# microsoft/StemGNN

Measured on AMD Instinct MI355X. Metric: forecast-steps/sec (train), higher is better.
Workload: dtype f32

## Files before the change

### stemgnn_amd/csrc/block.hip

```cpp
#include <hip/hip_runtime.h>

#include "../../include/stemgnn_hip.h"
#include "devattr.h"
#include "gemm2.h"
#include "gemm2s.h"
#include "gemm_core.h"
#include "layout.h"
#include "reduce.h"
#include "wgrad.h"
#include "heads.h"
#include "glu_fused.h"
#include "glu_fused_bf16.h"

#define SG_TRY(e)                                \
  do {                                           \
    hipError_t _e = (e);                         \
    if (_e != hipSuccess) return -(int)_e;       \
  } while (0)

__device__ __forceinline__ float sg_sigmoid(float v) { return __frcp_rn(1.f + __expf(-v)); }

struct SgDiv {
  unsigned d, magic;
  __device__ __forceinline__ int div(int x) const { return d == 1u ? x : (int)__umulhi((unsigned)x, magic); }
  __device__ __forceinline__ void divmod(int x, int& q, int& r) const { q = div(x); r = x - q * (int)d; }
};
static inline SgDiv sg_div(int d) {
  SgDiv v;
  v.d = (unsigned)d;
  v.magic = d > 1 ? (unsigned)((1ull << 32) / (unsigned)d + 1ull) : 0u;
  return v;
}
static inline bool sg_div_ok(long xmax, int d) { return d >= 1 && xmax >= 0 && (unsigned long long)xmax * (unsigned)d < (1ull << 32); }

struct XView {
  const float* p;
  long sb, sn, st;
  int N;
  __device__ __forceinline__ float at(int b, int n, int t) const { return p[b * sb + n * sn + t * st]; }
  __device__ __forceinline__ float row(int m, int t) const {
    const int b = m / N;
    return at(b, m - b * N, t);
  }
};

struct GftFwdOp {
  const float* T;
  XView X;
  float* G;
  int B, N, W;
  SgDiv dN, dW;
  __device__ bool setup(int, int& M, int& Nn, int& K0, int& K1) const {
    M = 3 * N; Nn = B * W; K0 = 0; K1 = N;
    return true;
  }
  __device__ float a(int, int i, int k) const { return T[(size_t)i * N + k]; }
  __device__ float b(int, int k, int j) const {
    int bb, t;
    dW.divmod(j, bb, t);
    return X.at(bb, k, t);
  }
  __device__ void epi(int, int i, int j, float v) const {
    int kq, n, bb, t;
    dN.divmod(i, kq, n);
    dW.divmod(j, bb, t);
    G[((size_t)bb * N + n) * (3 * W) + kq * W + t] = v;
  }
};

struct GftBwdDxOp {
  const float* T;
  const float* dG;
  float* dX;
  int B, N, W;
  size_t slab;
  SgDiv dN, dW;
  __device__ bool setup(int, int& M, int& Nn, int& K0, int& K1) const {
    M = N; Nn = B * W; K0 = 0; K1 = 3 * N;
    return true;
  }
  __device__ float a(int, int i, int k) const { return T[(size_t)k * N + i]; }
  __device__ float b(int, int k, int j) const {
    int kq, n, bb, t;
    dN.divmod(k, kq, n);
    dW.divmod(j, bb, t);
    const size_t o = ((size_t)bb * N + n) * (3 * W) + kq * W + t;
    return dG[o] + dG[o + slab];
  }
  __device__ void epi(int, int i, int j, float v) const {
    int bb, t;
    dW.divmod(j, bb, t);
    dX[((size_t)bb * N + i) * W + t] = v;
  }
};

struct GftBwdDtOp {
  const float* dG;
  XView X;
  float* dT;
  int B, N, W, accumulate;
  size_t slab;
  SgDiv dN, dW;
  __device__ bool setup(int, int& M, int& Nn, int& K0, int& K1) const {
    M = 3 * N; Nn = N; K0 = 0; K1 = B * W;
    return true;
  }
  __device__ float a(int, int i, int k) const {
    int kq, n, bb, t;
    dN.divmod(i, kq, n);
    dW.divmod(k, bb, t);
    const size_t o = ((size_t)bb * N + n) * (3 * W) + kq * W + t;
    return dG[o] + dG[o + slab];
  }
  __device__ float b(int, int k, int j) const {
    int bb, t;
    dW.divmod(k, bb, t);
    return X.at(bb, j, t);
  }
  __device__ void epi(int, int i, int j, float v) const {
    float* o = dT + (size_t)i * N + j;
    *o = accumulate ? (*o + v) : v;
  }
};

struct GftBwdDt2Op {
  const float* dG[2];
  XView X[2];
  float* dT;
  int B, N, W;
  size_t slab;
  SgDiv dN, dW;
  __device__ bool setup(int, int& M, int& Nn, int& K0, int& K1) const {
    M = 3 * N; Nn = N; K0 = 0; K1 = 2 * B * W;
    return true;
  }
  __device__ float a(int, int i, int k) const {
    const int blk = k >= B * W ? 1 : 0, kk = k - blk * B * W;
    int kq, n, bb, t;
    dN.divmod(i, kq, n);
    dW.divmod(kk, bb, t);
    const size_t o = ((size_t)bb * N + n) * (3 * W) + kq * W + t;
    const float* g = dG[blk];
    return g[o] + g[o + slab];
  }
  __device__ float b(int, int k, int j) const {
    const int blk = k >= B * W ? 1 : 0, kk = k - blk * B * W;
    int bb, t;
    dW.divmod(kk, bb, t);
    return X[blk].at(bb, j, t);
  }
  __device__ void epi(int, int i, int j, float v) const { dT[(size_t)i * N + j] = v; }
};

template <bool GATE = true>
struct GluFwdEpiT {
  static constexpr bool WHOLE = true;
  const float* bp[2];
  float* out[2];
  float* gate[2];
  int cp[2];
  template <int NI>
  __device__ void whole(int r, int, int row0, int col0, int M, int N, const sg_f32x16 (&acc)[NI][2], int lane) const {
    const bool hi = (lane & 16) != 0;
    const int k = lane & 15;
    const bool live0 = col0 < N, live1 = col0 + 32 < N;
    const float* b = bp[r];
    const float bl0 = live0 ? b[col0 + k] : 0.f, br0 = live0 ? b[col0 + 16 + k] : 0.f;
    const float bl1 = live1 ? b[col0 + 32 + k] : 0.f, br1 = live1 ? b[col0 + 48 + k] : 0.f;
    const bool live = hi ? live1 : live0;
    const int c = (col0 >> 1) + (lane & 31);
    float* po = out[r] + c;
    float* pg = GATE ? gate[r] + c : nullptr;
    const int ld = cp[r];
#pragma unroll
    for (int i = 0; i < NI; ++i) {
#pragma unroll
      for (int reg = 0; reg < 16; ++reg) {
        const float m0 = acc[i][0][reg], m1 = acc[i][1][reg];
        const float o0 = __shfl_xor(m0, 16, 64), o1 = __shfl_xor(m1, 16, 64);
        const float u = hi ? o1 + bl1 : m0 + bl0;
        const float v = hi ? m1 + br1 : o0 + br0;
        const float g = sg_sigmoid(v);
        const int row = row0 + i * 32 + g2_row_of(reg, lane);
        if (live && row < M) {
          po[(size_t)row * ld] = u * g;
          if constexpr (GATE) pg[(size_t)row * ld] = g;
        }
      }
    }
  }
};
using GluFwdEpi = GluFwdEpiT<true>;

struct GluDpreEpi {
  static constexpr bool WHOLE = true;
  const float* out[2];
  const float* gate[2];
  float* dpre[2];
  int cp;
  template <int NI>
  __device__ void whole(int r, int, int row0, int col0, int M, int N, const sg_f32x16 (&acc)[NI][2], int lane) const {
    const bool hi = (lane & 16) != 0;
    const float* po = out[r];
    const float* pg = gate[r];
    float* pd = dpre[r];
#pragma unroll
    for (int i = 0; i < NI; ++i) {
      float y[2][16], g[2][16];
#pragma unroll
      for (int j = 0; j < 2; ++j) {
        const int c = col0 + j * 32 + (lane & 31);
        const bool cl = c < N;
#pragma unroll
        for (int reg = 0; reg < 16; ++reg) {
          const int row = row0 + i * 32 + g2_row_of(reg, lane);
          const size_t o = (size_t)(row < M ? row : 0) * cp + (cl ? c : 0);
          y[j][reg] = po[o];
          g[j][reg] = pg[o];
        }
      }
#pragma unroll
      for (int j = 0; j < 2; ++j) {
        const int cb = col0 + j * 32;
        const bool cl = cb + (lane & 31) < N;
        const bool cl_lo = cb < N, cl_hi = cb + 16 < N;
        float* dp = pd + 2 * cb + (lane & 31);
#pragma unroll
        for (int reg = 0; reg < 16; ++reg) {
          const int row = row0 + i * 32 + g2_row_of(reg, lane);
          const float d = acc[i][j][reg];
          const float left = d * g[j][reg], right = d * y[j][reg] * (1.f - g[j][reg]);
          const float recv = __shfl_xor(hi ? left : right, 16, 64);
          if (row < M) {
            float* q = dp + (size_t)row * 2 * cp;
// ... 145 lines not shown
  __device__ float a(int, int i, int k) const {
    const float* p = k < Wm ? dpF + (size_t)i * Wm + k : dpB + (size_t)i * W + (k - Wm);
    return *p;
  }
  __device__ float b(int, int k, int j) const {
    const float* p = k < Wm ? Fw + (size_t)k * Wm + j : BCw + (size_t)(k - Wm) * Wm + j;
    return *p;
  }
  __device__ void epi(int, int i, int j, float v) const { dig[(size_t)i * Wm + j] = v; }
};

struct Da3Op {
  const float* dig;
  const float* wfold;
  const float* out[2];
  const float* gate[2];
  float* dpre[2];
  int cp2[2];
  int M, Wm, WmP;
  __device__ bool setup(int z, int& M_, int& N_, int& K0, int& K1) const {
    M_ = M; N_ = cp2[z]; K0 = 0; K1 = Wm;
    return true;
  }
  __device__ float a(int, int i, int k) const { return dig[(size_t)i * Wm + k]; }
  __device__ float b(int z, int k, int j) const { return wfold[(size_t)((z ? cp2[0] : 0) + j) * WmP + k]; }
  __device__ void epi(int z, int i, int j, float v) const {
    const size_t o = (size_t)i * cp2[z] + j;
    const float g = gate[z][o], y = out[z][o];
    float* dp = dpre[z] + (size_t)i * 2 * cp2[z] + ((j >> 4) << 5) + (j & 15);
    dp[0] = v * g;
    dp[16] = v * y * (1.f - g);
  }
};

struct HeadsWgradOp {
  const float *pa0[5], *pa1[5];
  int lda0[5], lda1[5], split[5], Mw[5], Nw[5], nb[5], rdiv[5], ldp[5], on[5];
  float sign[5];
  const float* pb[5];
  long sb[5], sn[5], st[5];
  float* part[5];
  int M, S, chunk;
  __device__ bool setup(int z, int& M_, int& N_, int& K0, int& K1) const {
    const int which = z / S, s = z - which * S;
    K0 = s * chunk; K1 = min(M, K0 + chunk);
    M_ = Mw[which]; N_ = Nw[which];
    return on[which] != 0;
  }
  __device__ float a(int z, int i, int k) const {
    const int w = z / S;
    const float *p0 = pa0[w], *p1 = pa1[w];
    const int l0 = lda0[w], l1 = lda1[w], sp = split[w];
    const float sg = sign[w];
    const bool lo = i < sp;
    const float* base = lo ? p0 : p1;
    const size_t off = (size_t)k * (lo ? l0 : l1) + (lo ? i : i - sp);
    return sg * base[off];
  }
  __device__ float b(int z, int k, int j) const {
    const int w = z / S;
    const int n = nb[w];
    const int kb = k / rdiv[w], kr = k - kb * rdiv[w];
    const float v = pb[w][kb * sb[w] + kr * sn[w] + (j < n ? j : n - 1) * st[w]];
    return j < n ? v : 1.f;
  }
  __device__ void epi(int z, int i, int j, float v) const {
    const int w = z / S, s = z - w * S;
    part[w][((size_t)s * Mw[w] + i) * ldp[w] + j] = v;
  }
};

constexpr int SG_LONG_K = 640;
constexpr int SG_WG_MAX_TILES = 256;
static inline bool wg_tiles_fit(WgGemm* q, int n) { return wg_tile_index(q, n) <= SG_WG_MAX_TILES; }
static inline int split_chunk(int M, int S) { return ((M + S - 1) / S + 15) & ~15; }

extern "C" int stemgnn_gft_fwd(const float* mul_L, const float* X, long xs_b, long xs_n, long xs_t,
                               float* G, int B, int N, int W, void* stream) {
  if (!mul_L || !X || !G || B <= 0 || N <= 0 || W <= 0) return SG_EINVAL;
  if (!sg_div_ok(3L * N + 64, N) || !sg_div_ok((long)B * W + 64, W)) return SG_EINVAL;
  GftFwdOp op{mul_L + (size_t)N * N, XView{X, xs_b, xs_n, xs_t, N}, G, B, N, W, sg_div(N), sg_div(W)};
  hipStream_t st = (hipStream_t)stream;
  if (N <= 512) {
    if (xs_n == 1) SG_TRY((sg_launch_gemm<GftFwdOp, 32, 32, true, true, false, 128, true>(op, 3 * N, B * W, 1, st)));
    else SG_TRY((sg_launch_gemm<GftFwdOp, 32, 32, true, false, false, 128, true>(op, 3 * N, B * W, 1, st)));
    return 0;
  }
  if (xs_n == 1) SG_TRY((sg_launch_gemm<GftFwdOp, 32, 64, true, true, false, 64, true>(op, 3 * N, B * W, 1, st)));
  else SG_TRY((sg_launch_gemm<GftFwdOp, 32, 64, true, false, false, 64, true>(op, 3 * N, B * W, 1, st)));
  return 0;
}

extern "C" int stemgnn_gft_bwd(const float* mul_L, const float* X, long xs_b, long xs_n, long xs_t,
                               const float* dG, float* dX, float* dmul_L, int accumulate,
                               int B, int N, int W, void* stream) {
  if (!mul_L || !X || !dG || (!dmul_L && !dX) || B <= 0 || N <= 0 || W <= 0) return SG_EINVAL;
  hipStream_t st = (hipStream_t)stream;
  const bool bk128 = N <= 512;
  if (!sg_div_ok(3L * N + 128, N) || !sg_div_ok((long)B * W + 128, W)) return SG_EINVAL;
  if (dX) {
    GftBwdDxOp op{mul_L + (size_t)N * N, dG, dX, B, N, W, (size_t)B * N * 3 * W, sg_div(N), sg_div(W)};
    if (bk128) SG_TRY((sg_launch_gemm<GftBwdDxOp, 32, 32, false, false, false, 128, true>(op, N, B * W, 1, st)));
    else SG_TRY((sg_launch_gemm<GftBwdDxOp, 32, 32, false, false, false, 64, true>(op, N, B * W, 1, st)));
  }
  if (!dmul_L) return 0;
  GftBwdDtOp op{dG, XView{X, xs_b, xs_n, xs_t, N}, dmul_L + (size_t)N * N, B, N, W, accumulate, (size_t)B * N * 3 * W, sg_div(N),
                sg_div(W)};
  if (bk128) {
    if (xs_t == 1) SG_TRY((sg_launch_gemm<GftBwdDtOp, 32, 32, true, true, false, 128, true>(op, 3 * N, N, 1, st)));
    else SG_TRY((sg_launch_gemm<GftBwdDtOp, 32, 32, true, false, false, 128, true>(op, 3 * N, N, 1, st)));
    return 0;
  }
  if (xs_t == 1) SG_TRY((sg_launch_gemm<GftBwdDtOp, 32, 32, true, true, false, 64, true>(op, 3 * N, N, 1, st)));
  else SG_TRY((sg_launch_gemm<GftBwdDtOp, 32, 32, true, false, false, 64, true>(op, 3 * N, N, 1, st)));
  return 0;
}

extern "C" int stemgnn_gft_bwd_dt2(const float* X0, long xs0_b, long xs0_n, long xs0_t, const float* dG0, const float* X1,
                                   long xs1_b, long xs1_n, long xs1_t, const float* dG1, float* dmul_L, int B, int N, int W,
                                   void* stream) {
  if (!X0 || !dG0 || !X1 || !dG1 || !dmul_L || B <= 0 || N <= 0 || W <= 0) return SG_EINVAL;
  hipStream_t st = (hipStream_t)stream;
  if (!sg_div_ok(3L * N + 128, N) || !sg_div_ok(2L * B * W + 128, W)) return SG_EINVAL;
  GftBwdDt2Op op{{dG0, dG1}, {XView{X0, xs0_b, xs0_n, xs0_t, N}, XView{X1, xs1_b, xs1_n, xs1_t, N}}, dmul_L + (size_t)N * N,
                 B, N, W, (size_t)B * N * 3 * W, sg_div(N), sg_div(W)};
  if (N <= 512) SG_TRY((sg_launch_gemm<GftBwdDt2Op, 32, 32, true, false, false, 128, true>(op, 3 * N, N, 1, st)));
  else SG_TRY((sg_launch_gemm<GftBwdDt2Op, 32, 32, true, false, false, 64, true>(op, 3 * N, N, 1, st)));
  return 0;
}

struct GluFwdBufs {
  const float* G;
  float* out[2][3];
  float* gate[2][3];
};
static GluFwdBufs glu_bufs_saved(const SgDims& d, float* saved) {
  const SgSavedLayout S = sg_saved_layout(d);
  GluFwdBufs b;
  b.G = saved + S.G;
  for (int r = 0; r < 2; ++r)
    for (int l = 0; l < 3; ++l) { b.out[r][l] = saved + S.out[r][l]; b.gate[r][l] = saved + S.gate[r][l]; }
  return b;
}
static GluFwdBufs glu_bufs_infer(const SgDims& d, float* ws, bool pp) {
  const SgInferLayout I = sg_infer_layout(d, pp);
  GluFwdBufs b;
  b.G = ws + I.G;
  for (int r = 0; r < 2; ++r) {
    b.out[r][0] = pp ? ws + I.pp[r][0] : nullptr;
    b.out[r][1] = pp ? ws + I.pp[r][1] : nullptr;
    b.out[r][2] = ws + I.out2[r];
    for (int l = 0; l < 3; ++l) b.gate[r][l] = nullptr;
  }
  return b;
}
template <bool INF>
static int glu_fwd_layers(const SgDims& d, const float* packed, const unsigned short* const* fpl, int splits,
                          const GluFwdBufs& bf, hipStream_t st) {
  const SgPackedLayout P = sg_packed_layout(d);
  using Epi = GluFwdEpiT<!INF>;
  for (int l = 0; l < 3; ++l) {
    G2Args g;
    G2SArgs gs;
    Epi e;
    for (int r = 0; r < 2; ++r) {
      g.A[r] = l == 0 ? bf.G : bf.out[r][l - 1];
      g.lda[r] = l == 0 ? d.KG : d.CP;
      g.B[r] = packed + P.w[r][l];
      g.ldb[r] = sg_glu_np(d, l, r);
      g.M[r] = d.M; g.N[r] = sg_glu_np(d, l, r); g.K[r] = sg_glu_kin(d, l);
      if (fpl) {
        gs.A[r] = g.A[r]; gs.lda[r] = g.lda[r]; gs.P[r] = fpl[r * 3 + l];
        gs.M[r] = g.M[r]; gs.N[r] = g.N[r]; gs.K[r] = g.K[r]; gs.Kp[r] = g2s_pad32(g.K[r]);
      }
      e.bp[r] = packed + P.b[r][l];
      e.out[r] = bf.out[r][l];
      e.gate[r] = bf.gate[r][l];
      e.cp[r] = sg_glu_cp(d, l, r);
    }
    g.nsplit = 1; g.chunk = (sg_glu_kin(d, l) + 15) & ~15; g.b_ones_col = -1;
    if (fpl && l > 0 && g2s_ok(gs, 2)) {
      SG_TRY((g2s_launch<Epi>(gs, e, 2, splits, st)));
      continue;
    }
    if (sg_glu_kin(d, l) > SG_LONG_K) SG_TRY((g2_launch<Epi, true, false, 64, true>(g, e, 2, st)));
    else SG_TRY((g2_launch<Epi, true, false, 64>(g, e, 2, st)));
  }
  return 0;
}

static int glu_fused_mode() {
  const char* ef = getenv("STEMGNN_GLU_FUSED");
  return ef ? atoi(ef) : 1;
}
static inline bool sg_aligned16(const void* p) { return (((uintptr_t)p) & 15) == 0; }
static bool glu_fwd_fused_ok(const SgDims& d, int fmode, const void* packed) {
  return gf_geom(d).ok && fmode != 0 && sg_aligned16(packed);
}
static bool glu_dgrad_fused_ok(const SgDims& d, int dmode, const void* packed, const void* scratch) {
  return gd_geom(d).ok && dmode != 0 && sg_aligned16(packed) && sg_aligned16(scratch);
}

template <bool INF = false>
static int glu_fwd_impl(const float* packed, const GluFwdBufs& bf, int B, int N, int W, int multi, void* stream, int m_pick,
                        bool fused_only) {
  if (!packed || !bf.G || B <= 0 || N <= 0 || W <= 0 || multi <= 0) return SG_EINVAL;
  const SgDims d = sg_dims(B, N, W, multi);
  const SgPackedLayout P = sg_packed_layout(d);
// ... 790 lines not shown
```

### stemgnn_amd/csrc/front.hip

```cpp
#include <hip/hip_runtime.h>
#include <stdlib.h>
#include <stdint.h>

#include "../../include/stemgnn_hip.h"
#include "dq_reduce.h"
#include "gemm_core.h"
#include "layout.h"

#define SG_TRY(e)                                \
  do {                                           \
    hipError_t _e = (e);                         \
    if (_e != hipSuccess) return -(int)_e;       \
  } while (0)

constexpr int ATTN_NBC = 8;

__device__ __forceinline__ void sg_philox4(uint64_t seed, uint64_t offset, uint64_t idx, uint32_t (&w)[4]) {
  uint32_t c0 = (uint32_t)idx, c1 = (uint32_t)(idx >> 32), c2 = (uint32_t)offset, c3 = (uint32_t)(offset >> 32);
  uint32_t k0 = (uint32_t)seed, k1 = (uint32_t)(seed >> 32);
#pragma unroll
  for (int r = 0; r < 10; ++r) {
    const uint32_t hi0 = __umulhi(0xD2511F53u, c0), lo0 = 0xD2511F53u * c0;
    const uint32_t hi1 = __umulhi(0xCD9E8D57u, c2), lo1 = 0xCD9E8D57u * c2;
    c0 = hi1 ^ c1 ^ k0; c1 = lo1; c2 = hi0 ^ c3 ^ k1; c3 = lo0;
    k0 += 0x9E3779B9u; k1 += 0xBB67AE85u;
  }
  w[0] = c0; w[1] = c1; w[2] = c2; w[3] = c3;
}
__device__ __forceinline__ int sg_drop_nq(int N) { return 64 * ((N + 255) >> 8); }
__device__ __forceinline__ bool sg_keep_word(uint32_t w, float p) { return (float)w * 2.3283064365386963e-10f >= p; }

__device__ __forceinline__ float sg_wave_sum(float v) {
#pragma unroll
  for (int o = 32; o > 0; o >>= 1) v += __shfl_xor(v, o, 64);
  return v;
}
__device__ __forceinline__ float sg_wave_max(float v) {
#pragma unroll
  for (int o = 32; o > 0; o >>= 1) v = fmaxf(v, __shfl_xor(v, o, 64));
  return v;
}
__device__ __forceinline__ float sg_lrelu(float v, float alpha) { return v > 0.f ? v : alpha * v; }

__global__ __launch_bounds__(256) void sg_keyquery_kernel(const float* __restrict__ h, const float* __restrict__ wk,
                                                          const float* __restrict__ wq, float* __restrict__ key,
                                                          float* __restrict__ query, int B, int N) {
  __shared__ float red[4][64][2];
  const int b = blockIdx.x, lane = threadIdx.x & 63, wave = threadIdx.x >> 6;
  const int i = blockIdx.y * 64 + lane;
  float ak = 0.f, aq = 0.f;
  if (i < N) {
    const float* hp = h + (size_t)b * N + i;
    const size_t stride = (size_t)B * N;
#pragma unroll 4
    for (int s = wave; s < N; s += 4) {
      const float v = hp[s * stride];
      ak = fmaf(v, wk[s], ak);
      aq = fmaf(v, wq[s], aq);
    }
  }
  red[wave][lane][0] = ak;
  red[wave][lane][1] = aq;
  __syncthreads();
  if (wave == 0 && i < N) {
    key[(size_t)b * N + i] = (red[0][lane][0] + red[1][lane][0]) + (red[2][lane][0] + red[3][lane][0]);
    query[(size_t)b * N + i] = (red[0][lane][1] + red[1][lane][1]) + (red[2][lane][1] + red[3][lane][1]);
  }
}

__global__ __launch_bounds__(256) void sg_attention_fwd_kernel(
    const float* __restrict__ key, const float* __restrict__ query, float alpha, float drop_p, int training,
    const uint64_t* __restrict__ seedp, int B, int N, int bn, float* __restrict__ rowsum, float* __restrict__ Apart,
    float* __restrict__ degpart) {
  extern __shared__ __attribute__((aligned(16))) float smem[];
  float* qmax = smem;
  const int lane = threadIdx.x & 63, wave = threadIdx.x >> 6;
  float* acc = smem + bn + wave * N;
  const int b0 = blockIdx.y * bn, b1 = min(B, b0 + bn);
  for (int b = b0 + wave; b < b1; b += 4) {
    float m = -INFINITY;
    for (int j = lane; j < N; j += 64) m = fmaxf(m, query[(size_t)b * N + j]);
    m = sg_wave_max(m);
    if (lane == 0) qmax[b - b0] = m;
  }
  __syncthreads();
  const int i = blockIdx.x * 4 + wave;
  if (i >= N) return;
  const bool drop = training && drop_p > 0.f;
  uint64_t seed = 0, offset = 0;
// ... 414 lines not shown
  __shared__ float red[4][2];
  const int s = blockIdx.x;
  const size_t BN = (size_t)B * N;
  float ak = 0.f, aq = 0.f;
  for (size_t e = threadIdx.x; e < BN; e += 256) {
    const float hv = h[(size_t)s * BN + e];
    ak = fmaf(dkey[e], hv, ak);
    aq = fmaf(dquery[e], hv, aq);
  }
  ak = sg_wave_sum(ak);
  aq = sg_wave_sum(aq);
  const int lane = threadIdx.x & 63, wave = threadIdx.x >> 6;
  if (lane == 0) { red[wave][0] = ak; red[wave][1] = aq; }
  __syncthreads();
  if (threadIdx.x == 0) {
    dwk[s] = (red[0][0] + red[1][0]) + (red[2][0] + red[3][0]);
    dwq[s] = (red[0][1] + red[1][1]) + (red[2][1] + red[3][1]);
  }
}

__global__ void sg_dropout_mask_kernel(float drop_p, const uint64_t* __restrict__ seedp, size_t n, int N, float* __restrict__ mask) {
  const size_t idx = (size_t)blockIdx.x * blockDim.x + threadIdx.x;
  if (idx >= n) return;
  const size_t row = idx / (size_t)N;
  const int j = (int)(idx - row * (size_t)N);
  uint32_t w[4];
  sg_philox4(seedp[0], seedp[1], row * sg_drop_nq(N) + (uint64_t)((j >> 8) * 64 + (j & 63)), w);
  mask[idx] = sg_keep_word(w[(j >> 6) & 3], drop_p) ? 1.f : 0.f;
}

struct ChebFwdOp {
  const float* L;
  const float* Bm;
  float* out;
  int N, sub;
  __device__ bool setup(int, int& M, int& Nn, int& K0, int& K1) const {
    M = N; Nn = N; K0 = 0; K1 = N;
    return true;
  }
  __device__ float a(int, int i, int k) const { return L[(size_t)i * N + k]; }
  __device__ float b(int, int k, int j) const { return Bm[(size_t)k * N + j]; }
  __device__ void epi(int, int i, int j, float v) const {
    const size_t o = (size_t)i * N + j;
    out[o] = sub ? 2.f * v - L[o] : 2.f * v;
  }
};

struct ChebBwd1Op {
  const float *L, *T2, *dT1, *dT2, *dT3;
  float *dLp, *dT2p;
  int N;
  __device__ bool setup(int, int& M, int& Nn, int& K0, int& K1) const {
    M = N; Nn = N; K0 = 0; K1 = N;
    return true;
  }
  __device__ float a(int z, int i, int k) const { return z == 0 ? dT3[(size_t)i * N + k] : L[(size_t)k * N + i]; }
  __device__ float b(int z, int k, int j) const { return z == 0 ? T2[(size_t)j * N + k] : dT3[(size_t)k * N + j]; }
  __device__ void epi(int z, int i, int j, float v) const {
    const size_t o = (size_t)i * N + j;
    if (z == 0) dLp[o] = dT1[o] - dT3[o] + 2.f * v;
    else dT2p[o] = dT2[o] + 2.f * v;
  }
};
struct ChebBwd2Op {
  const float *L, *dT2p, *dLp;
  float* dL;
  int N;
  __device__ bool setup(int, int& M, int& Nn, int& K0, int& K1) const {
    M = N; Nn = N; K0 = 0; K1 = 2 * N;
    return true;
  }
  __device__ float a(int, int i, int k) const {
    const float* p = k < N ? dT2p + (size_t)i * N + k : L + (size_t)(k - N) * N + i;
    return *p;
  }
  __device__ float b(int, int k, int j) const {
    const float* p = k < N ? L + (size_t)j * N + k : dT2p + (size_t)(k - N) * N + j;
    return *p;
  }
  __device__ void epi(int, int i, int j, float v) const {
    const size_t o = (size_t)i * N + j;
    dL[o] = dLp[o] + 2.f * v;
  }
};

extern "C" size_t stemgnn_attn_saved_floats(int B, int N) {
  return (size_t)3 * B * N + (size_t)N * N + N + (size_t)ATTN_NBC * N * N + (size_t)ATTN_NBC * N + B;
}
extern "C" size_t stemgnn_attn_scratch_floats(int B, int N, int nchunk) {
  return (size_t)N * N + (size_t)2 * B * N + (size_t)B * nchunk * N;
}

extern "C" int stemgnn_attn_laplacian_fwd(const float* h, const float* wk, const float* wq, float alpha,
                                          float drop_p, int training, const uint64_t* seed, int B, int N,
                                          float* saved, float* attention_out, float* mul_L, int parts, void* stream) {
  if (!h || !wk || !wq || !saved || !attention_out || !mul_L || B <= 0 || N <= 0 || (parts & 3) == 0) return SG_EINVAL;
  if (training && drop_p > 0.f && !seed) return SG_EINVAL;
  if (drop_p < 0.f || drop_p >= 1.f) return SG_EINVAL;
  hipStream_t st = (hipStream_t)stream;
  float* key = saved;
  float* query = key + (size_t)B * N;
  float* rowsum = query + (size_t)B * N;
  float* A = rowsum + (size_t)B * N;
  float* deg = A + (size_t)N * N;
  if (parts & 1) {
    hipLaunchKernelGGL(sg_keyquery_kernel, dim3(B, (N + 63) / 64), dim3(256), 0, st, h, wk, wq, key, query, B, N);
    SG_TRY(hipGetLastError());
    float* Apart = deg + N;
    float* degpart = Apart + (size_t)ATTN_NBC * N * N;
    const int nbc = B < ATTN_NBC ? B : ATTN_NBC;
    const int bn = (B + nbc - 1) / nbc;
    const size_t lds = (size_t)(bn + 4 * N) * sizeof(float);
    if (lds > 64 * 1024) return SG_EINVAL;
    hipLaunchKernelGGL(sg_attention_fwd_kernel, dim3((N + 3) / 4, (B + bn - 1) / bn), dim3(256), lds, st, key, query, alpha,
                       drop_p, training, seed, B, N, bn, rowsum, Apart, degpart);
    SG_TRY(hipGetLastError());
    if (parts & 2) {
      hipLaunchKernelGGL(sg_laplacian_fused_kernel, dim3((N + 31) / 32, (N + 31) / 32), dim3(256), 0, st, Apart, degpart,
                         (B + bn - 1) / bn, B, N, A, deg, attention_out, mul_L);
      SG_TRY(hipGetLastError());
      return 0;
    }
    hipLaunchKernelGGL(sg_attention_reduce_kernel, dim3((N + 3) / 4), dim3(256), 0, st, Apart, (B + bn - 1) / bn, B, N, A, deg);
    SG_TRY(hipGetLastError());
  }
  if (parts & 2) {
    hipLaunchKernelGGL(sg_laplacian_fwd_kernel, dim3((N + 31) / 32, (N + 31) / 32), dim3(256), 0, st, A, deg,
                       attention_out, mul_L, N);
    SG_TRY(hipGetLastError());
  }
  return 0;
}

extern "C" int stemgnn_attn_laplacian_bwd(const float* dL, const float* h, const float* wk, const float* wq,
                                          float alpha, float drop_p, int training, const uint64_t* seed, int B, int N,
                                          const float* saved, float* scratch, int nchunk, float* dh, float* dwk,
                                          float* dwq, int parts, void* stream) {
  const bool factored = (parts & 4) != 0;
  if (!dL || !h || !wk || !wq || !saved || !scratch || ((parts & 2) && !factored && (!dh || !dwk || !dwq)) || B <= 0 ||
      N <= 0 || nchunk <= 0 || (parts & 3) == 0)
    return SG_EINVAL;
  if (training && drop_p > 0.f && !seed) return SG_EINVAL;
  hipStream_t st = (hipStream_t)stream;
  const float* key = saved;
  const float* query = key + (size_t)B * N;
  const float* rowsum = query + (size_t)B * N;
  const float* A = rowsum + (size_t)B * N;
  const float* deg = A + (size_t)N * N;
  float* dAB = scratch;
  float* dkey = dAB + (size_t)N * N;
  float* dquery = dkey + (size_t)B * N;
  float* dqpart = dquery + (size_t)B * N;
  if (parts & 1) {
    hipLaunchKernelGGL(sg_laplacian_bwd_kernel, dim3((N + 3) / 4), dim3(256), 0, st, dL, A, deg, dAB, B, N,
                       (training && drop_p > 0.f) ? 1 : 0);
    SG_TRY(hipGetLastError());
  }
  if (!(parts & 2)) return 0;
  const size_t lds = (size_t)(4 * N) * sizeof(float);
  if (lds > 150 * 1024) return SG_EINVAL;
  hipLaunchKernelGGL(sg_attention_bwd_kernel, dim3(B, nchunk), dim3(256), lds, st, dAB, key, query, rowsum, alpha,
                     drop_p, training, seed, B, N, nchunk, dkey, dqpart);
  SG_TRY(hipGetLastError());
  if ((parts & 8) && factored) return 0;
  {
    const size_t bn = (size_t)B * N;
// ... 5 lines not shown
  hipLaunchKernelGGL(sg_keyquery_bwd_kernel, dim3(N), dim3(256), 0, st, h, wk, wq, dkey, dquery, dh, dwk, dwq, B, N);
  SG_TRY(hipGetLastError());
  return 0;
}

extern "C" int stemgnn_attn_dquery_reduce(float* attn_scratch, int B, int N, int nchunk, float* out, void* stream) {
  if (!attn_scratch || B <= 0 || N <= 0 || nchunk <= 0) return SG_EINVAL;
  float* dquery = attn_scratch + (size_t)N * N + (size_t)B * N;
  const size_t bn = (size_t)B * N;
  hipLaunchKernelGGL(sg_dquery_reduce_kernel, dim3((unsigned)((bn + 255) / 256)), dim3(256), 0, (hipStream_t)stream,
                     dquery + bn, out ? out : dquery, B, N, nchunk);
  SG_TRY(hipGetLastError());
  return 0;
}
extern "C" int stemgnn_keyquery_wgrad2(const float* h, const float* dkey, const float* dquery, float* dwk, float* dwq, int B,
                                       int N, void* stream) {
  if (!h || !dkey || !dquery || !dwk || !dwq || B <= 0 || N <= 0) return SG_EINVAL;
  hipLaunchKernelGGL(sg_keyquery_wgrad_kernel, dim3(N), dim3(256), 0, (hipStream_t)stream, h, dkey, dquery, dwk, dwq, B, N);
  SG_TRY(hipGetLastError());
  return 0;
}

extern "C" int stemgnn_keyquery_wgrad(const float* h, const float* attn_scratch, float* dwk, float* dwq, int B, int N,
                                      void* stream) {
  if (!h || !attn_scratch || !dwk || !dwq || B <= 0 || N <= 0) return SG_EINVAL;
  const float* dkey = attn_scratch + (size_t)N * N;
  hipLaunchKernelGGL(sg_keyquery_wgrad_kernel, dim3(N), dim3(256), 0, (hipStream_t)stream, h, dkey, dkey + (size_t)B * N, dwk,
                     dwq, B, N);
  SG_TRY(hipGetLastError());
  return 0;
}

__global__ void sg_dropout_seed_next_kernel(uint64_t* __restrict__ seed, uint64_t* __restrict__ used) {
  if (threadIdx.x == 0 && blockIdx.x == 0) {
    const uint64_t key = seed[0], off = seed[1];
    used[0] = key;
    used[1] = off;
    seed[1] = off + 1;
  }
}
extern "C" int stemgnn_dropout_seed_next(uint64_t* seed, uint64_t* used, void* stream) {
  if (!seed || !used || seed == used) return SG_EINVAL;
  hipLaunchKernelGGL(sg_dropout_seed_next_kernel, dim3(1), dim3(64), 0, (hipStream_t)stream, seed, used);
  SG_TRY(hipGetLastError());
  return 0;
}

extern "C" int stemgnn_dropout_mask(float drop_p, const uint64_t* seed, int B, int N, float* mask, void* stream) {
  if (!seed || !mask || B <= 0 || N <= 0) return SG_EINVAL;
  const size_t n = (size_t)B * N * N;
  hipLaunchKernelGGL(sg_dropout_mask_kernel, dim3((unsigned)((n + 255) / 256)), dim3(256), 0, (hipStream_t)stream,
                     drop_p, seed, n, N, mask);
  SG_TRY(hipGetLastError());
  return 0;
}

extern "C" int stemgnn_cheb_fwd(float* mul_L, int N, void* stream) {
  if (!mul_L || N <= 0) return SG_EINVAL;
  hipStream_t st = (hipStream_t)stream;
  const size_t nn = (size_t)N * N;
  float* L = mul_L + nn;
  ChebFwdOp op2{L, L, mul_L + 2 * nn, N, 0};
  if (N <= 512) {
    SG_TRY((sg_launch_gemm<ChebFwdOp, 32, 32, true, false, false, 128, true>(op2, N, N, 1, st)));
    ChebFwdOp op3b{L, mul_L + 2 * nn, mul_L + 3 * nn, N, 1};
    SG_TRY((sg_launch_gemm<ChebFwdOp, 32, 32, true, false, false, 128, true>(op3b, N, N, 1, st)));
    return 0;
  }
  SG_TRY((sg_launch_gemm<ChebFwdOp, 32, 32, true, false, false, 64, true>(op2, N, N, 1, st)));
  ChebFwdOp op3{L, mul_L + 2 * nn, mul_L + 3 * nn, N, 1};
  SG_TRY((sg_launch_gemm<ChebFwdOp, 32, 32, true, false, false, 64, true>(op3, N, N, 1, st)));
  return 0;
}

extern "C" int stemgnn_cheb_bwd(const float* mul_L, const float* dmul_L, float* dL, float* scratch, int N,
                                void* stream) {
  if (!mul_L || !dmul_L || !dL || !scratch || N <= 0) return SG_EINVAL;
  hipStream_t st = (hipStream_t)stream;
  const size_t nn = (size_t)N * N;
  float* dLp = scratch;
  float* dT2p = scratch + nn;
  ChebBwd1Op op1{mul_L + nn, mul_L + 2 * nn, dmul_L + nn, dmul_L + 2 * nn, dmul_L + 3 * nn, dLp, dT2p, N};
  if (N <= 512) {
    SG_TRY((sg_launch_gemm<ChebBwd1Op, 32, 32, true, true, false, 128, true>(op1, N, N, 2, st)));
    ChebBwd2Op op2b{mul_L + nn, dT2p, dLp, dL, N};
    SG_TRY((sg_launch_gemm<ChebBwd2Op, 32, 32, true, true, false, 128, true>(op2b, N, N, 1, st)));
    return 0;
  }
  SG_TRY((sg_launch_gemm<ChebBwd1Op, 32, 32, true, true, false, 64, true>(op1, N, N, 2, st)));
  ChebBwd2Op op2{mul_L + nn, dT2p, dLp, dL, N};
  SG_TRY((sg_launch_gemm<ChebBwd2Op, 32, 32, true, true, false, 64, true>(op2, N, N, 1, st)));
  return 0;
}
```

Measured before the change: 84840.

## Add phased GEMM kernel with compile-time index maps for GFT and Chebyshev paths

Adds a new 32x32-tile MFMA GEMM kernel whose operands use templated integer row/column offset functions and per-phase K ranges. GFT forward, GFT backward dX, GFT backward dT2, and Chebyshev backward step 1 use it for N<=512 by default; an environment variable turns it off. The goal is cheaper address arithmetic (32-bit offsets, layout-specialised coalesced loads) and less runtime branching on block index in the inner loop than the generic gemm launcher. The cost is extra code paths, overflow guards that limit it to tensors under 2^31 elements, and possibly worse tiling than the tuned generic kernel.

```diff
diff --git a/stemgnn_amd/csrc/block.hip b/stemgnn_amd/csrc/block.hip
--- a/stemgnn_amd/csrc/block.hip
+++ b/stemgnn_amd/csrc/block.hip
@@ -5,6 +5,7 @@
 #include "gemm2.h"
 #include "gemm2s.h"
 #include "gemm_core.h"
+#include "gemm_phased.h"
 #include "layout.h"
 #include "reduce.h"
 #include "wgrad.h"
@@ -150,6 +151,103 @@
     return X[blk].at(bb, j, t);
   }
   __device__ void epi(int, int i, int j, float v) const { dT[(size_t)i * N + j] = v; }
+};
+
+struct XViewI {
+  const float* p;
+  int sb, sn, st;
+};
+static inline bool sg_phased_fits(int B, int N, int W, long xs_b, long xs_n, long xs_t) {
+  if (xs_b < 0 || xs_n < 0 || xs_t < 0) return false;
+  const long lim = 1L << 31;
+  if (xs_b >= lim || xs_n >= lim || xs_t >= lim) return false;
+  return 2L * B * N * 3 * W < lim && (B - 1) * xs_b + (N - 1) * xs_n + (W - 1) * xs_t < lim;
+}
+
+template <bool XKF>
+struct GftFwdPhOp {
+  static constexpr int NZ = 1, NPH = 1;
+  template <int Z, int P> static constexpr bool akf() { return true; }
+  template <int Z, int P> static constexpr bool bkf() { return XKF; }
+  GftFwdOp o;
+  XViewI X;
+  __device__ bool setup(int, int& M, int& Nn, int& K) const {
+    M = 3 * o.N; Nn = o.B * o.W; K = o.N;
+    return true;
+  }
+  template <int Z, int P> __device__ int arow(int i) const { return i * o.N; }
+  template <int Z, int P> __device__ int acol(int k) const { return k; }
+  template <int Z, int P> __device__ float aval(int off) const { return o.T[off]; }
+  template <int Z, int P> __device__ int brow(int k) const { return k * X.sn; }
+  template <int Z, int P> __device__ int bcol(int j) const {
+    int bb, t;
+    o.dW.divmod(j, bb, t);
+    return bb * X.sb + t * X.st;
+  }
+  template <int Z, int P> __device__ float bval(int off) const { return X.p[off]; }
+  __device__ void epi(int z, int i, int j, float v) const { o.epi(z, i, j, v); }
+};
+
+struct GftBwdDxPhOp {
+  static constexpr int NZ = 1, NPH = 1;
+  template <int Z, int P> static constexpr bool akf() { return false; }
+  template <int Z, int P> static constexpr bool bkf() { return false; }
+  GftBwdDxOp o;
+  __device__ bool setup(int, int& M, int& Nn, int& K) const {
+    M = o.N; Nn = o.B * o.W; K = 3 * o.N;
+    return true;
+  }
+  template <int Z, int P> __device__ int arow(int i) const { return i; }
+  template <int Z, int P> __device__ int acol(int k) const { return k * o.N; }
+  template <int Z, int P> __device__ float aval(int off) const { return o.T[off]; }
+  template <int Z, int P> __device__ int brow(int k) const {
+    int kq, n;
+    o.dN.divmod(k, kq, n);
+    return n * (3 * o.W) + kq * o.W;
+  }
+  template <int Z, int P> __device__ int bcol(int j) const {
+    int bb, t;
+    o.dW.divmod(j, bb, t);
+    return bb * (o.N * 3 * o.W) + t;
+  }
+  template <int Z, int P> __device__ float bval(int off) const { return o.dG[off] + o.dG[off + o.slab]; }
+  __device__ void epi(int z, int i, int j, float v) const { o.epi(z, i, j, v); }
+};
+
+template <bool X0KF, bool X1KF>
+struct GftBwdDt2PhOp {
+  static constexpr int NZ = 1, NPH = 2;
+  template <int Z, int P> static constexpr bool akf() { return true; }
+  template <int Z, int P> static constexpr bool bkf() { return P == 0 ? X0KF : X1KF; }
+  GftBwdDt2Op o;
+  XViewI X[2];
+  __device__ bool setup(int, int& M, int& Nn, int& K) const {
+    M = 3 * o.N; Nn = o.N; K = 2 * o.B * o.W;
+    return true;
+  }
+  __device__ int pend() const { return o.B * o.W; }
+  template <int Z, int P> __device__ int arow(int i) const {
+    int kq, n;
+    o.dN.divmod(i, kq, n);
+    return n * (3 * o.W) + kq * o.W;
+  }
+  template <int Z, int P> __device__ int acol(int k) const {
+    int bb, t;
+    o.dW.divmod(k - P * o.B * o.W, bb, t);
+    return bb * (o.N * 3 * o.W) + t;
+  }
+  template <int Z, int P> __device__ float aval(int off) const {
+    const float* g = o.dG[P];
+    return g[off] + g[off + o.slab];
+  }
+  template <int Z, int P> __device__ int brow(int k) const {
+    int bb, t;
+    o.dW.divmod(k - P * o.B * o.W, bb, t);
+    return bb * X[P].sb + t * X[P].st;
+  }
+  template <int Z, int P> __device__ int bcol(int j) const { return j * X[P].sn; }
+  template <int Z, int P> __device__ float bval(int off) const { return X[P].p[off]; }
+  __device__ void epi(int z, int i, int j, float v) const { o.epi(z, i, j, v); }
 };
 
 template <bool GATE = true>
@@ -461,6 +559,12 @@
   GftFwdOp op{mul_L + (size_t)N * N, XView{X, xs_b, xs_n, xs_t, N}, G, B, N, W, sg_div(N), sg_div(W)};
   hipStream_t st = (hipStream_t)stream;
   if (N <= 512) {
+    if (sg_graph_phased() && sg_phased_fits(B, N, W, xs_b, xs_n, xs_t)) {
+      const XViewI xi{X, (int)xs_b, (int)xs_n, (int)xs_t};
+      if (xs_n == 1) SG_TRY((sg_launch_phased<GftFwdPhOp<true>>(GftFwdPhOp<true>{op, xi}, 3 * N, B * W, st)));
+      else SG_TRY((sg_launch_phased<GftFwdPhOp<false>>(GftFwdPhOp<false>{op, xi}, 3 * N, B * W, st)));
+      return 0;
+    }
     if (xs_n == 1) SG_TRY((sg_launch_gemm<GftFwdOp, 32, 32, true, true, false, 128, true>(op, 3 * N, B * W, 1, st)));
     else SG_TRY((sg_launch_gemm<GftFwdOp, 32, 32, true, false, false, 128, true>(op, 3 * N, B * W, 1, st)));
     return 0;
@@ -479,7 +583,9 @@
   if (!sg_div_ok(3L * N + 128, N) || !sg_div_ok((long)B * W + 128, W)) return SG_EINVAL;
   if (dX) {
     GftBwdDxOp op{mul_L + (size_t)N * N, dG, dX, B, N, W, (size_t)B * N * 3 * W, sg_div(N), sg_div(W)};
-    if (bk128) SG_TRY((sg_launch_gemm<GftBwdDxOp, 32, 32, false, false, false, 128, true>(op, N, B * W, 1, st)));
+    if (bk128 && sg_graph_phased() && sg_phased_fits(B, N, W, 0, 0, 0))
+      SG_TRY((sg_launch_phased<GftBwdDxPhOp>(GftBwdDxPhOp{op}, N, B * W, st)));
+    else if (bk128) SG_TRY((sg_launch_gemm<GftBwdDxOp, 32, 32, false, false, false, 128, true>(op, N, B * W, 1, st)));
     else SG_TRY((sg_launch_gemm<GftBwdDxOp, 32, 32, false, false, false, 64, true>(op, N, B * W, 1, st)));
   }
   if (!dmul_L) return 0;
@@ -503,6 +609,15 @@
   if (!sg_div_ok(3L * N + 128, N) || !sg_div_ok(2L * B * W + 128, W)) return SG_EINVAL;
   GftBwdDt2Op op{{dG0, dG1}, {XView{X0, xs0_b, xs0_n, xs0_t, N}, XView{X1, xs1_b, xs1_n, xs1_t, N}}, dmul_L + (size_t)N * N,
                  B, N, W, (size_t)B * N * 3 * W, sg_div(N), sg_div(W)};
+  if (N <= 512 && sg_graph_phased() && sg_phased_fits(B, N, W, xs0_b, xs0_n, xs0_t) && sg_phased_fits(B, N, W, xs1_b, xs1_n, xs1_t)) {
+    const XViewI x0{X0, (int)xs0_b, (int)xs0_n, (int)xs0_t}, x1{X1, (int)xs1_b, (int)xs1_n, (int)xs1_t};
+    const bool k0 = xs0_t == 1, k1 = xs1_t == 1;
+    if (k0 && k1) SG_TRY((sg_launch_phased<GftBwdDt2PhOp<true, true>>(GftBwdDt2PhOp<true, true>{op, {x0, x1}}, 3 * N, N, st)));
+    else if (k0) SG_TRY((sg_launch_phased<GftBwdDt2PhOp<true, false>>(GftBwdDt2PhOp<true, false>{op, {x0, x1}}, 3 * N, N, st)));
+    else if (k1) SG_TRY((sg_launch_phased<GftBwdDt2PhOp<false, true>>(GftBwdDt2PhOp<false, true>{op, {x0, x1}}, 3 * N, N, st)));
+    else SG_TRY((sg_launch_phased<GftBwdDt2PhOp<false, false>>(GftBwdDt2PhOp<false, false>{op, {x0, x1}}, 3 * N, N, st)));
+    return 0;
+  }
   if (N <= 512) SG_TRY((sg_launch_gemm<GftBwdDt2Op, 32, 32, true, false, false, 128, true>(op, 3 * N, N, 1, st)));
   else SG_TRY((sg_launch_gemm<GftBwdDt2Op, 32, 32, true, false, false, 64, true>(op, 3 * N, N, 1, st)));
   return 0;
diff --git a/stemgnn_amd/csrc/front.hip b/stemgnn_amd/csrc/front.hip
--- a/stemgnn_amd/csrc/front.hip
+++ b/stemgnn_amd/csrc/front.hip
@@ -5,6 +5,7 @@
 #include "../../include/stemgnn_hip.h"
 #include "dq_reduce.h"
 #include "gemm_core.h"
+#include "gemm_phased.h"
 #include "layout.h"
 
 #define SG_TRY(e)                                \
@@ -585,6 +586,24 @@
     const size_t o = (size_t)i * N + j;
     dL[o] = dLp[o] + 2.f * v;
   }
+};
+
+struct ChebBwd1PhOp {
+  static constexpr int NZ = 2, NPH = 1;
+  template <int Z, int P> static constexpr bool akf() { return Z == 0; }
+  template <int Z, int P> static constexpr bool bkf() { return Z == 0; }
+  ChebBwd1Op o;
+  __device__ bool setup(int, int& M, int& Nn, int& K) const {
+    M = o.N; Nn = o.N; K = o.N;
+    return true;
+  }
+  template <int Z, int P> __device__ int arow(int i) const { return Z == 0 ? i * o.N : i; }
+  template <int Z, int P> __device__ int acol(int k) const { return Z == 0 ? k : k * o.N; }
+  template <int Z, int P> __device__ float aval(int off) const { return (Z == 0 ? o.dT3 : o.L)[off]; }
+  template <int Z, int P> __device__ int brow(int k) const { return Z == 0 ? k : k * o.N; }
+  template <int Z, int P> __device__ int bcol(int j) const { return Z == 0 ? j * o.N : j; }
+  template <int Z, int P> __device__ float bval(int off) const { return (Z == 0 ? o.T2 : o.dT3)[off]; }
+  __device__ void epi(int z, int i, int j, float v) const { o.epi(z, i, j, v); }
 };
 
 extern "C" size_t stemgnn_attn_saved_floats(int B, int N) {
@@ -756,8 +775,9 @@
   float* dT2p = scratch + nn;
   ChebBwd1Op op1{mul_L + nn, mul_L + 2 * nn, dmul_L + nn, dmul_L + 2 * nn, dmul_L + 3 * nn, dLp, dT2p, N};
   if (N <= 512) {
-    SG_TRY((sg_launch_gemm<ChebBwd1Op, 32, 32, true, true, false, 128, true>(op1, N, N, 2, st)));
     ChebBwd2Op op2b{mul_L + nn, dT2p, dLp, dL, N};
+    if (sg_graph_phased()) SG_TRY((sg_launch_phased<ChebBwd1PhOp>(ChebBwd1PhOp{op1}, N, N, st)));
+    else SG_TRY((sg_launch_gemm<ChebBwd1Op, 32, 32, true, true, false, 128, true>(op1, N, N, 2, st)));
     SG_TRY((sg_launch_gemm<ChebBwd2Op, 32, 32, true, true, false, 128, true>(op2b, N, N, 1, st)));
     return 0;
   }
diff --git a/stemgnn_amd/csrc/gemm_phased.h b/stemgnn_amd/csrc/gemm_phased.h
--- /dev/null
+++ b/stemgnn_amd/csrc/gemm_phased.h
@@ -0,0 +1,186 @@
+#pragma once
+#include <stdlib.h>
+
+#include "gemm_core.h"
+
+template <int I>
+struct sg_ic {
+  static constexpr int value = I;
+};
+
+template <class Op, int BK, int Z>
+__device__ __forceinline__ void sg_phased_body(const Op& op, float* lds) {
+  constexpr int NPH = Op::NPH;
+  static_assert(NPH == 1 || NPH == 2, "phases");
+  static_assert(BK % 16 == 0 && (BK & (BK - 1)) == 0, "BK");
+  constexpr bool LAST_AKF = Op::template akf<Z, NPH - 1>(), LAST_BKF = Op::template bkf<Z, NPH - 1>();
+  constexpr int SA = 32 + ((Op::template akf<Z, 0>() || LAST_AKF) ? 17 : 16);
+  constexpr int SB = 32 + ((Op::template bkf<Z, 0>() || LAST_BKF) ? 17 : 16);
+  constexpr int R = 32 * BK / 256;
+  float* As = lds;
+  float* Bs = lds + BK * 49;
+
+  int M, N, K;
+  if (!op.setup(Z, M, N, K)) return;
+  const int m0 = blockIdx.x * 32;
+  const int n0 = blockIdx.y * 32;
+  if (m0 >= M || n0 >= N) return;
+  int pb[NPH + 1];
+  pb[0] = 0;
+  pb[NPH] = K;
+  if constexpr (NPH == 2) pb[1] = op.pend();
+
+  const int tid = threadIdx.x;
+  const int lane = tid & 63;
+  const int wave = tid >> 6;
+  const int wm = wave >> 1, wn = wave & 1;
+
+  sg_f32x4 acc = (sg_f32x4){0.f, 0.f, 0.f, 0.f}, acc2 = (sg_f32x4){0.f, 0.f, 0.f, 0.f};
+  float ra[R], rb[R];
+
+  auto gload = [&](auto pc, int kb) {
+    constexpr int P = decltype(pc)::value;
+    const int lo = pb[P], hi = pb[P + 1];
+    auto ck = [&](int gk) { return gk < lo ? lo : (gk < hi ? gk : hi - 1); };
+    if constexpr (Op::template akf<Z, P>()) {
+      const int gk = kb + tid % BK;
+      const int co = op.template acol<Z, P>(ck(gk));
+      const bool kin = gk >= lo && gk < hi;
+#pragma unroll
+      for (int r = 0; r < R; ++r) {
+        const int gi = m0 + tid / BK + (256 / BK) * r;
+        const float v = op.template aval<Z, P>(op.template arow<Z, P>(gi < M ? gi : M - 1) + co);
+        ra[r] = (gi < M && kin) ? v : 0.f;
+      }
+    } else {
+      const int gi = m0 + (tid & 31);
+      const int ro = op.template arow<Z, P>(gi < M ? gi : M - 1);
+#pragma unroll
+      for (int r = 0; r < R; ++r) {
+        const int gk = kb + (tid >> 5) + 8 * r;
+        const float v = op.template aval<Z, P>(ro + op.template acol<Z, P>(ck(gk)));
+        ra[r] = (gi < M && gk >= lo && gk < hi) ? v : 0.f;
+      }
+    }
+    if constexpr (Op::template bkf<Z, P>()) {
+      const int gk = kb + tid % BK;
+      const int ro = op.template brow<Z, P>(ck(gk));
+      const bool kin = gk >= lo && gk < hi;
+#pragma unroll
+      for (int r = 0; r < R; ++r) {
+        const int gj = n0 + tid / BK + (256 / BK) * r;
+        const float v = op.template bval<Z, P>(ro + op.template bcol<Z, P>(gj < N ? gj : N - 1));
+        rb[r] = (gj < N && kin) ? v : 0.f;
+      }
+    } else {
+      const int gj = n0 + (tid & 31);
+      const int co = op.template bcol<Z, P>(gj < N ? gj : N - 1);
+#pragma unroll
+      for (int r = 0; r < R; ++r) {
+        const int gk = kb + (tid >> 5) + 8 * r;
+        const float v = op.template bval<Z, P>(op.template brow<Z, P>(ck(gk)) + co);
+        rb[r] = (gj < N && gk >= lo && gk < hi) ? v : 0.f;
+      }
+    }
+  };
+  auto lstore = [&](auto pc, int kb) {
+    constexpr int P = decltype(pc)::value;
+    const int lo = pb[P], hi = pb[P + 1];
+    auto mine = [&](int gk) { return (P == 0 || gk >= lo) && (P == NPH - 1 || gk < hi); };
+    if constexpr (Op::template akf<Z, P>()) {
+      const int k = tid % BK;
+      if (mine(kb + k)) {
+#pragma unroll
+        for (int r = 0; r < R; ++r) As[k * SA + tid / BK + (256 / BK) * r] = ra[r];
+      }
+    } else {
+#pragma unroll
+      for (int r = 0; r < R; ++r) {
+        const int k = (tid >> 5) + 8 * r;
+        if (mine(kb + k)) As[k * SA + (tid & 31)] = ra[r];
+      }
+    }
+    if constexpr (Op::template bkf<Z, P>()) {
+      const int k = tid % BK;
+      if (mine(kb + k)) {
+#pragma unroll
+        for (int r = 0; r < R; ++r) Bs[k * SB + tid / BK + (256 / BK) * r] = rb[r];
+      }
+    } else {
+#pragma unroll
+      for (int r = 0; r < R; ++r) {
+        const int k = (tid >> 5) + 8 * r;
+        if (mine(kb + k)) Bs[k * SB + (tid & 31)] = rb[r];
+      }
+    }
+  };
+
+  const int fi = lane & 15;
+  const int fk = lane >> 4;
+
+  auto phase = [&](auto pc) {
+    constexpr int P = decltype(pc)::value;
+    constexpr bool LAST = P == NPH - 1;
+    using Next = sg_ic<LAST ? P : P + 1>;
+    const int hi = pb[P + 1];
+    for (int kb = pb[P] & ~(BK - 1); kb < hi; kb += BK) {
+      lstore(pc, kb);
+      if constexpr (!LAST) {
+        if (kb + BK > hi) {
+          gload(Next{}, kb);
+          break;
+        }
+      }
+      __syncthreads();
+      if (kb + BK < hi) gload(pc, kb + BK);
+      else if constexpr (!LAST) gload(Next{}, kb + BK);
+#pragma unroll
+      for (int ks = 0; ks < BK; ks += 4) {
+        const float af = As[(ks + fk) * SA + wm * 16 + fi];
+        const float bf = Bs[(ks + fk) * SB + wn * 16 + fi];
+        acc = __builtin_amdgcn_mfma_f32_16x16x4f32(af, bf, acc, 0, 0, 0);
+      }
+      acc2 += acc;
+      acc = (sg_f32x4){0.f, 0.f, 0.f, 0.f};
+      __syncthreads();
+    }
+  };
+
+  gload(sg_ic<0>{}, 0);
+  phase(sg_ic<0>{});
+  if constexpr (NPH == 2) phase(sg_ic<1>{});
+
+  const int gj = n0 + wn * 16 + fi;
+#pragma unroll
+  for (int reg = 0; reg < 4; ++reg) {
+    const int gi = m0 + wm * 16 + fk * 4 + reg;
+    if (gi < M && gj < N) op.epi(Z, gi, gj, acc2[reg]);
+  }
+}
+
+template <class Op, int BK>
+__global__ __launch_bounds__(256) void sg_gemm_phased_f32(const Op op) {
+  static_assert(Op::NZ == 1 || Op::NZ == 2, "z");
+  __builtin_amdgcn_s_setprio(SG_CHAIN_PRIO);
+  __shared__ float lds[2 * BK * 49];
+  if constexpr (Op::NZ == 2) {
+    if (blockIdx.z == 1) {
+      sg_phased_body<Op, BK, 1>(op, lds);
+      return;
+    }
+  }
+  sg_phased_body<Op, BK, 0>(op, lds);
+}
+
+template <class Op, int BK = 128>
+static inline hipError_t sg_launch_phased(const Op& op, int maxM, int maxN, hipStream_t stream) {
+  dim3 grid((maxM + 31) / 32, (maxN + 31) / 32, Op::NZ);
+  if (grid.x == 0 || grid.y == 0) return hipSuccess;
+  hipLaunchKernelGGL((sg_gemm_phased_f32<Op, BK>), grid, dim3(256), 0, stream, op);
+  return hipGetLastError();
+}
+
+static inline bool sg_graph_phased() {
+  const char* e = getenv("STEMGNN_GRAPH_PHASED");
+  return !(e && e[0] == '0' && e[1] == '\0');
+}
```

After: 85750, median of 6. +1.1%, better.
